# nicolapiccinelli/libmpc

Measured on AMD Instinct MI355X. Metric: MPC solves/sec (whole node) + p50 solve latency, quadrotor LMPC N=20 batch=4096, higher is better.
Workload: dtype f64; 1 GPU; quadrotor_ex.cpp LMPC nx=12 nu=4 ny=12 ph=ch=20, batch 4096 per GPU, SplitMix64 x0/u0/yref (SURVEY 8d), maximum_iteration=250; parallelism=single GPU, rccl_ranks=0, streams=1

## Files before the change

### include/mpcx.h

```cpp
#ifndef MPCX_H
#define MPCX_H

#include <stdint.h>

#ifdef __cplusplus
extern "C" {
#endif

#define MPCX_OK              0
#define MPCX_E_INVALID      -1
#define MPCX_E_UNSUPPORTED  -2
#define MPCX_E_DEVICE       -3
#define MPCX_E_NUMERIC      -4
#define MPCX_E_STATE        -5

#define MPCX_STATUS_SUCCESS        0
#define MPCX_STATUS_MAX_ITERATION  1
#define MPCX_STATUS_INFEASIBLE     2
#define MPCX_STATUS_ERROR          3
#define MPCX_STATUS_UNKNOWN        4

#define MPCX_SOLVER_SOLVED               1
#define MPCX_SOLVER_SOLVED_INACCURATE    2
#define MPCX_SOLVER_MAX_ITER_REACHED    -2
// ... 348 lines not shown
int mpcx_comm_get_unique_id(void *id_out );
int mpcx_comm_create(int device, int rank, int world, const void *id, mpcx_comm_t *out);
int mpcx_comm_destroy(mpcx_comm_t c);
int mpcx_comm_rank(mpcx_comm_t c);
int mpcx_comm_world(mpcx_comm_t c);
int mpcx_allgather_u(mpcx_comm_t c, const double *u_local, int rows_per_rank, int nu, double *u_all, void *stream);

typedef struct mpcx_lmpc_hetero *mpcx_lmpc_hetero_t;
int mpcx_lmpc_hetero_create(const mpcx_lmpc_t *controllers, int count, int device, mpcx_lmpc_hetero_t *out);
int mpcx_lmpc_hetero_create_ex(const mpcx_lmpc_t *controllers, int count, int device, int condense_on_host, mpcx_lmpc_hetero_t *out);
int mpcx_lmpc_hetero_destroy(mpcx_lmpc_hetero_t f);
int mpcx_lmpc_hetero_get_info(mpcx_lmpc_hetero_t f, int *count, int *active_words, int *m_ref, double *bytes_per_model);
int mpcx_lmpc_hetero_solve_batch(mpcx_lmpc_hetero_t f, const mpcx_lmpc_batch *b, const int32_t *model_index, void *stream);
int mpcx_lmpc_hetero_time_solve_batch(mpcx_lmpc_hetero_t f, const mpcx_lmpc_batch *b, const int32_t *model_index, void *stream,
                                      int repeats, float *ms_mean);
int mpcx_lmpc_hetero_sensitivity_batch(mpcx_lmpc_hetero_t f, const mpcx_lmpc_sens *s, const int32_t *model_index, void *stream);
int mpcx_lmpc_hetero_loop_create(mpcx_lmpc_hetero_t f, const mpcx_lmpc_loop_desc *d, const int32_t *model_index, void *stream, mpcx_lmpc_loop_t *out);
int mpcx_lmpc_hetero_loop_create_observed(mpcx_lmpc_hetero_t f, const mpcx_lmpc_loop_desc *d, const mpcx_lmpc_observer_desc *o, const int32_t *model_index,
                                          void *stream, mpcx_lmpc_loop_t *out);
int mpcx_lmpc_hetero_loop_create_offset_free(mpcx_lmpc_hetero_t f, const mpcx_lmpc_loop_desc *d, const mpcx_lmpc_disturbance_observer_desc *o,
                                             const int32_t *model_index, void *stream, mpcx_lmpc_loop_t *out);
int mpcx_lmpc_hetero_loop_create_offset_free_target(mpcx_lmpc_hetero_t f, const mpcx_lmpc_loop_desc *d, const mpcx_lmpc_disturbance_observer_desc *o,
                                                    const mpcx_lmpc_target_desc *t, const int32_t *model_index, void *stream, mpcx_lmpc_loop_t *out);

int mpcx_lmpc_set_total_batch(mpcx_lmpc_t h, int total);

int mpcx_lmpc_debug_time_kernels(mpcx_lmpc_t h, const mpcx_lmpc_batch *b, void *stream, int repeats, float *ms3);
int mpcx_lmpc_debug_get(mpcx_lmpc_t h, const char *name, double *out, int cap);
int mpcx_lmpc_debug_setup_counts(mpcx_lmpc_t h, int *full, int *refs);
int mpcx_lmpc_debug_use_fused(mpcx_lmpc_t h, int mode);
int mpcx_lmpc_debug_force_generic(mpcx_lmpc_t h, int on);
int mpcx_lmpc_debug_set_rounds(mpcx_lmpc_t h, int rounds0, int check_every);
int mpcx_lmpc_debug_set_cycle_buffer(mpcx_lmpc_t h, void *dev_ptr);
int mpcx_lmpc_loop_debug_replay(mpcx_lmpc_loop_t l, void *stream);
int mpcx_lmpc_loop_debug_tick(mpcx_lmpc_loop_t l, int *tick);
int mpcx_nlmpc_loop_debug_replay(mpcx_nlmpc_loop_t l, void *stream);
int mpcx_nlmpc_loop_debug_tick(mpcx_nlmpc_loop_t l, int *tick);
int mpcx_nlmpc_debug_set_tolerances(mpcx_nlmpc_t h, double tol_step, double tol_con);
int mpcx_nlmpc_debug_last_form(void);
int mpcx_dare_debug_product(int product);
int mpcx_nlmpc_last_form(mpcx_nlmpc_t h);
int mpcx_nlmpc_debug_get_ws(mpcx_nlmpc_t h, int instance, double *out, int cap, int *layout, int nlayout);
int mpcx_nlmpc_debug_generated_source(const mpcx_nlmpc_source *src, char *out, int cap);
int mpcx_nlmpc_debug_compile_source(const mpcx_nlmpc_source *src);
int mpcx_lmpc_hetero_debug_get(mpcx_lmpc_hetero_t f, int k, const char *name, double *out, int cap);

const char *mpcx_version(void);

#ifdef __cplusplus
}
#endif
#endif
```

### libmpc_amd/_capi.py

```python
from __future__ import annotations

import ctypes as C
import os

_HERE = os.path.dirname(os.path.abspath(__file__))
LIB_PATH = os.environ.get("MPCX_LIBRARY", os.path.join(_HERE, "libmpcx.so"))

OK = 0
E_INVALID, E_UNSUPPORTED, E_DEVICE, E_NUMERIC, E_STATE = -1, -2, -3, -4, -5
STATUS_SUCCESS, STATUS_MAX_ITERATION, STATUS_INFEASIBLE, STATUS_ERROR, STATUS_UNKNOWN = range(5)
REF_SHARED, REF_PER_INSTANCE, REF_PER_STEP = 0, 1, 2
DARE_CONTROL, DARE_ESTIMATOR = 0, 1
REF_PREVIEW = 3


class Dims(C.Structure):
    _fields_ = [(n, C.c_int) for n in ("nx", "nu", "ndu", "ny", "ph", "ch")]


class LParams(C.Structure):
    _fields_ = [("maximum_iteration", C.c_int), ("time_limit", C.c_double), ("enable_warm_start", C.c_int),
                ("alpha", C.c_double), ("rho", C.c_double), ("eps_rel", C.c_double), ("eps_abs", C.c_double),
                ("eps_prim_inf", C.c_double), ("eps_dual_inf", C.c_double),
                ("verbose", C.c_int), ("adaptive_rho", C.c_int), ("polish", C.c_int)]
# ... 78 lines not shown
    "mpcx_lmpc_set_objective_weights", "mpcx_lmpc_set_objective_weights_slice",
    "mpcx_lmpc_set_state_bounds", "mpcx_lmpc_set_state_bounds_slice",
    "mpcx_lmpc_set_input_bounds", "mpcx_lmpc_set_input_bounds_slice",
    "mpcx_lmpc_set_output_bounds", "mpcx_lmpc_set_output_bounds_slice",
    "mpcx_lmpc_set_input_rate_bounds", "mpcx_lmpc_set_input_rate_bounds_slice",
    "mpcx_lmpc_set_soft_constraint_weights", "mpcx_lmpc_set_soft_constraint_weights_slice",
    "mpcx_lmpc_set_terminal_cost",
    "mpcx_lmpc_set_linear_constraints", "mpcx_lmpc_set_linear_constraints_slice",
    "mpcx_lmpc_set_linear_constraint_weights", "mpcx_lmpc_set_linear_constraint_weights_slice",
    "mpcx_lmpc_set_scalar_constraint_slice", "mpcx_lmpc_set_scalar_constraint_index",
    "mpcx_lmpc_set_references", "mpcx_lmpc_set_references_slice",
    "mpcx_lmpc_set_exogenous_inputs", "mpcx_lmpc_set_exogenous_inputs_slice",
    "mpcx_lmpc_set_optimizer_parameters", "mpcx_lmpc_set_strict_infeasibility", "mpcx_lmpc_setup", "mpcx_lmpc_solve_batch",
    "mpcx_lmpc_time_solve_batch", "mpcx_lmpc_sensitivity_batch", "mpcx_lmpc_sens_size", "mpcx_lmpc_sensitivity_host",
    "mpcx_lmpc_param_sensitivity_batch", "mpcx_lmpc_param_sens_size", "mpcx_lmpc_param_sens_reserve", "mpcx_lmpc_param_sensitivity_host",
    "mpcx_lmpc_model_sensitivity_batch", "mpcx_lmpc_model_sens_size", "mpcx_lmpc_model_sens_reserve", "mpcx_lmpc_model_sensitivity_host", "mpcx_lmpc_solve_host", "mpcx_lmpc_get_info", "mpcx_version",
    "mpcx_lmpc_graph_create", "mpcx_lmpc_graph_launch", "mpcx_lmpc_graph_destroy",
    "mpcx_lmpc_loop_create", "mpcx_lmpc_loop_run", "mpcx_lmpc_loop_destroy", "mpcx_lmpc_loop_desc_size",
    "mpcx_lmpc_loop_create_observed", "mpcx_lmpc_hetero_loop_create_observed", "mpcx_lmpc_observer_desc_size", "mpcx_lmpc_kalman_gain",
    "mpcx_lmpc_loop_create_offset_free", "mpcx_lmpc_hetero_loop_create_offset_free", "mpcx_lmpc_disturbance_observer_desc_size",
    "mpcx_lmpc_loop_create_offset_free_target", "mpcx_lmpc_hetero_loop_create_offset_free_target", "mpcx_lmpc_target_desc_size",
    "mpcx_target_map_batch", "mpcx_target_apply_batch",
    "mpcx_nlmpc_create", "mpcx_nlmpc_destroy", "mpcx_nlmpc_get_dims", "mpcx_nlmpc_evaluate_batch",
    "mpcx_nlparams_default", "mpcx_nlmpc_set_optimizer_parameters", "mpcx_nlmpc_solve_batch", "mpcx_nlmpc_time_solve_batch", "mpcx_discretize_batch", "mpcx_dare_batch",
    "mpcx_nlmpc_set_state_bounds_slice", "mpcx_nlmpc_set_input_bounds_slice", "mpcx_nlmpc_solve_host",
    "mpcx_nlmpc_create_custom", "mpcx_nlmpc_create_from_source", "mpcx_nlmpc_set_input_scale", "mpcx_nlmpc_set_state_scale",
    "mpcx_nlmpc_loop_create", "mpcx_nlmpc_loop_run", "mpcx_nlmpc_loop_destroy", "mpcx_nlmpc_loop_desc_size", "mpcx_nlmpc_plant_step_batch",
    "mpcx_nlmpc_loop_create_observed", "mpcx_nlmpc_ekf_desc_size", "mpcx_nlmpc_ekf_step_batch",
    "mpcx_comm_get_unique_id", "mpcx_comm_create", "mpcx_comm_destroy", "mpcx_comm_rank", "mpcx_comm_world", "mpcx_allgather_u",
    "mpcx_lmpc_hetero_create", "mpcx_lmpc_hetero_destroy", "mpcx_lmpc_hetero_get_info", "mpcx_lmpc_hetero_solve_batch",
    "mpcx_lmpc_hetero_time_solve_batch", "mpcx_lmpc_hetero_create_ex", "mpcx_lmpc_hetero_debug_get", "mpcx_lmpc_hetero_loop_create",
    "mpcx_lmpc_hetero_sensitivity_batch",
    "mpcx_lmpc_set_total_batch", "mpcx_lmpc_debug_time_kernels", "mpcx_lmpc_debug_get", "mpcx_lmpc_debug_setup_counts", "mpcx_lmpc_debug_use_fused",
    "mpcx_lmpc_debug_force_generic", "mpcx_lmpc_debug_set_rounds", "mpcx_lmpc_debug_set_cycle_buffer",
    "mpcx_lmpc_loop_debug_replay", "mpcx_lmpc_loop_debug_tick", "mpcx_nlmpc_loop_debug_replay", "mpcx_nlmpc_loop_debug_tick",
    "mpcx_dare_debug_product", "mpcx_nlmpc_debug_set_tolerances", "mpcx_nlmpc_debug_last_form", "mpcx_nlmpc_last_form", "mpcx_nlmpc_debug_get_ws", "mpcx_nlmpc_debug_generated_source", "mpcx_nlmpc_debug_compile_source",
]


class NLParams(C.Structure):
    _fields_ = [("maximum_iteration", C.c_int), ("time_limit", C.c_double), ("enable_warm_start", C.c_int),
                ("relative_ftol", C.c_double), ("relative_xtol", C.c_double), ("absolute_ftol", C.c_double),
                ("absolute_xtol", C.c_double), ("hard_constraints", C.c_int)]


class NlmpcBatch(C.Structure):
    _fields_ = [("batch", C.c_int), ("x0", C.c_void_p), ("u0", C.c_void_p), ("z_warm", C.c_void_p), ("cmd", C.c_void_p),
                ("cost", C.c_void_p), ("status", C.c_void_p), ("solver_status", C.c_void_p), ("is_feasible", C.c_void_p),
                ("iterations", C.c_void_p), ("z", C.c_void_p), ("seq_state", C.c_void_p), ("seq_input", C.c_void_p),
                ("seq_output", C.c_void_p), ("warm_curvature", C.c_int), ("multipliers", C.c_void_p), ("params", C.c_void_p)]


class NlmpcLoopDesc(C.Structure):
    _fields_ = [("batch", C.c_int), ("ticks", C.c_int), ("x0", C.c_void_p), ("u0", C.c_void_p),
                ("params", C.c_void_p), ("plant_params", C.c_void_p), ("noise", C.c_void_p),
                ("substeps", C.c_int), ("warm", C.c_int),
                ("traj_x", C.c_void_p), ("traj_u", C.c_void_p), ("traj_cost", C.c_void_p),
                ("traj_status", C.c_void_p), ("traj_solver_status", C.c_void_p), ("traj_is_feasible", C.c_void_p),
                ("traj_iterations", C.c_void_p)]


class NlmpcEkfDesc(C.Structure):
    _fields_ = [("ny", C.c_int), ("Cm", C.c_void_p), ("Q", C.c_void_p), ("R", C.c_void_p), ("P0", C.c_void_p),
                ("xhat0", C.c_void_p), ("meas_noise", C.c_void_p), ("traj_xhat", C.c_void_p), ("traj_y", C.c_void_p),
                ("traj_P", C.c_void_p), ("ekf_flags", C.c_void_p)]


# ... 44 lines not shown
        _lib.mpcx_lmpc_hetero_sensitivity_batch.argtypes = [C.c_void_p] * 4
        _lib.mpcx_lmpc_param_sensitivity_batch.argtypes = [C.c_void_p] * 3
        _lib.mpcx_lmpc_param_sens_reserve.argtypes = [C.c_void_p, C.c_int]
        _lib.mpcx_lmpc_param_sensitivity_host.argtypes = [C.c_void_p] * 3 + [C.c_int] + [C.c_void_p] * 7
        _lib.mpcx_lmpc_model_sensitivity_batch.argtypes = [C.c_void_p] * 3
        _lib.mpcx_lmpc_model_sens_reserve.argtypes = [C.c_void_p, C.c_int]
        _lib.mpcx_lmpc_model_sensitivity_host.argtypes = [C.c_void_p] * 3 + [C.c_int] + [C.c_void_p] * 7
        _lib.mpcx_lmpc_graph_create.argtypes = [C.c_void_p, C.c_void_p, C.c_void_p, C.c_void_p]
        _lib.mpcx_lmpc_graph_launch.argtypes = [C.c_void_p, C.c_void_p]
        _lib.mpcx_lmpc_graph_destroy.argtypes = [C.c_void_p]
        _lib.mpcx_lmpc_loop_create.argtypes = [C.c_void_p, C.c_void_p, C.c_void_p, C.c_void_p]
        _lib.mpcx_lmpc_hetero_loop_create.argtypes = [C.c_void_p, C.c_void_p, C.c_void_p, C.c_void_p, C.c_void_p]
        _lib.mpcx_lmpc_loop_create_observed.argtypes = [C.c_void_p] * 5
        _lib.mpcx_lmpc_hetero_loop_create_observed.argtypes = [C.c_void_p] * 6
        _lib.mpcx_lmpc_loop_create_offset_free.argtypes = [C.c_void_p] * 5
        _lib.mpcx_lmpc_hetero_loop_create_offset_free.argtypes = [C.c_void_p] * 6
        _lib.mpcx_lmpc_loop_create_offset_free_target.argtypes = [C.c_void_p] * 6
        _lib.mpcx_lmpc_hetero_loop_create_offset_free_target.argtypes = [C.c_void_p] * 7
        _lib.mpcx_target_map_batch.argtypes = [C.c_int] * 6 + [C.c_void_p] * 9
        _lib.mpcx_target_apply_batch.argtypes = [C.c_int] * 5 + [C.c_void_p, C.c_int] + [C.c_void_p] * 5
        _lib.mpcx_lmpc_kalman_gain.argtypes = [C.c_void_p] * 6
        _lib.mpcx_lmpc_loop_run.argtypes = [C.c_void_p, C.c_void_p]
        _lib.mpcx_lmpc_loop_destroy.argtypes = [C.c_void_p]
        _lib.mpcx_lmpc_loop_debug_replay.argtypes = [C.c_void_p, C.c_void_p]
        _lib.mpcx_lmpc_loop_debug_tick.argtypes = [C.c_void_p, C.c_void_p]
        _lib.mpcx_nlmpc_get_dims.argtypes = [C.c_void_p, C.c_void_p]
        _lib.mpcx_nlmpc_evaluate_batch.argtypes = [C.c_void_p, C.c_int] + [C.c_void_p] * 9
        _lib.mpcx_nlparams_default.restype = None
        for _n in ("mpcx_nlmpc_set_state_bounds_slice", "mpcx_nlmpc_set_input_bounds_slice"):
            getattr(_lib, _n).argtypes = [C.c_void_p, C.c_void_p, C.c_void_p, C.c_int, C.c_int]
        _lib.mpcx_discretize_batch.argtypes = [C.c_int] * 4 + [C.c_void_p] * 3 + [C.c_int] + [C.c_void_p] * 3
        _lib.mpcx_dare_batch.argtypes = [C.c_int] * 5 + [C.c_void_p] * 4 + [C.c_int] * 2 + [C.c_void_p] * 5
        _lib.mpcx_dare_debug_product.argtypes = [C.c_int]
        _lib.mpcx_nlmpc_set_optimizer_parameters.argtypes = [C.c_void_p, C.c_void_p]
        _lib.mpcx_nlmpc_solve_batch.argtypes = [C.c_void_p, C.c_void_p, C.c_void_p]
        _lib.mpcx_nlmpc_time_solve_batch.argtypes = [C.c_void_p, C.c_void_p, C.c_void_p, C.c_int, C.c_void_p]
        _lib.mpcx_nlmpc_create_from_source.argtypes = [C.c_void_p, C.c_double, C.c_int, C.c_void_p]
        _lib.mpcx_nlmpc_set_input_scale.argtypes = [C.c_void_p, C.c_void_p]
        _lib.mpcx_nlmpc_set_state_scale.argtypes = [C.c_void_p, C.c_void_p]
        _lib.mpcx_nlmpc_loop_create.argtypes = [C.c_void_p, C.c_void_p, C.c_void_p, C.c_void_p]
        _lib.mpcx_nlmpc_loop_run.argtypes = [C.c_void_p, C.c_void_p]
        _lib.mpcx_nlmpc_loop_destroy.argtypes = [C.c_void_p]
        _lib.mpcx_nlmpc_loop_debug_replay.argtypes = [C.c_void_p, C.c_void_p]
        _lib.mpcx_nlmpc_loop_debug_tick.argtypes = [C.c_void_p, C.c_void_p]
        _lib.mpcx_nlmpc_plant_step_batch.argtypes = [C.c_void_p, C.c_int] + [C.c_void_p] * 4 + [C.c_int, C.c_void_p, C.c_void_p]
        _lib.mpcx_nlmpc_loop_create_observed.argtypes = [C.c_void_p] * 5
        _lib.mpcx_nlmpc_ekf_step_batch.argtypes = [C.c_void_p, C.c_int] + [C.c_void_p] * 8 + [C.c_int, C.c_int] + [C.c_void_p] * 4
        _lib.mpcx_comm_get_unique_id.argtypes = [C.c_void_p]
        _lib.mpcx_comm_create.argtypes = [C.c_int, C.c_int, C.c_int, C.c_void_p, C.c_void_p]
        _lib.mpcx_comm_destroy.argtypes = [C.c_void_p]
        _lib.mpcx_comm_rank.argtypes = [C.c_void_p]
        _lib.mpcx_comm_world.argtypes = [C.c_void_p]
        _lib.mpcx_allgather_u.argtypes = [C.c_void_p, C.c_void_p, C.c_int, C.c_int, C.c_void_p, C.c_void_p]
    return _lib


def check(rc):
    if rc < 0:
        raise MpcxError(rc, lib().mpcx_last_error().decode())
    return rc
```

### libmpc_amd/csrc/lmpc_device.hpp

```cpp
#pragma once

#include <atomic>
#include <cstdint>
#include <initializer_list>

namespace mpcx {

constexpr int kMaxActive = 28;
constexpr int kSld = kMaxActive + 1;
__host__ __device__ inline int ws_limit(int nz, int mg, int n_soft) { return nz + (n_soft < mg ? n_soft : mg); }
__host__ __device__ inline int ws_capacity(int limit) { return limit > kMaxActive ? limit : kMaxActive; }

struct LmpcDev {
    int nx, nu, ndu, ny, ph, ch, nf, nz, mg;
    int ldz, ldg, ldy;
    int m_ref, neq_ref, active_words;
    int has_dist, n_fixed;
    int max_iter, polish, check_every, polish_rounds0, polish_rounds;
    int cost_direct;
    int cond_status;
    int strict_infeasible;
    int n_soft;
    double alpha, sigma, eps_abs, eps_rel, eps_prim_inf;
    int adaptive_rho; double rho_user;
// ... 49 lines not shown
    const int32_t *model_index;
    long long *dbg_cycles;
};
static_assert(sizeof(LmpcDev) == 712 && sizeof(LmpcBatchDev) == 296, "LmpcDev / LmpcBatchDev changed size: see kernarg_touch (lmpc_fast.hip)");
__host__ __device__ inline size_t lmpc_slot_len(const LmpcDev &m) { const size_t n = (size_t)ws_limit(m.nz, m.mg, m.n_soft); return n * n; }
__host__ __device__ inline int lmpc_model_of(const LmpcBatchDev &Bt, int b) { return Bt.n_models <= 0 ? 0 : (Bt.model_index ? Bt.model_index[b] : b); }

constexpr int kFqCount = 0, kFqTicket = 1, kFqServed = 2, kFqList = 4;
inline size_t lmpc_fallback_queue_bytes(size_t cap) { return (kFqList + cap) * sizeof(int); }
int lmpc_fallback_waves();
int lmpc_fallback_reset(int *fq, void *stream);

size_t lmpc_lds_limit();
int lmpc_kernel_variant(int ldz, int ldg);
struct LmpcScratch { double *ws; size_t cap; int *fq; double *pbuf; int pslots; int *pcounter; };
int lmpc_scratch_reserve(LmpcScratch &s, const LmpcDev &m, int batch, bool with_pcounter, void *stream);
void lmpc_scratch_release(LmpcScratch &s);

enum class LmpcAssemble { Generic, MfmaSharedYref, MfmaInstanceYref };
enum class LmpcForm { TwoKernels, FusedMatvec, Group };
struct LmpcPlan {
    LmpcAssemble assemble;
    LmpcForm form;
    int fused;
};
int lmpc_launch(const LmpcDev &m, const LmpcDev *m_dev, const LmpcBatchDev &b, const LmpcScratch &scratch, void *stream, int which, const LmpcPlan &plan);
int lmpc_fallback_slots(const LmpcDev &m, int batch);
int lmpc_lds_per_wave(const LmpcDev &m, int *stage_len, int *arena_len);
void lmpc_pack_mfma_tiles(const double *src, int rows, int K, double *out);
inline size_t lmpc_packed_len(int rows, int K) { return (size_t)(rows / 16) * ((K + 15) / 16) * 256; }
int lmpc_fast_slice(const LmpcDev &m);
size_t lmpc_group_lds_bytes(const LmpcDev &m);
int lmpc_launch_fast(const LmpcDev &m, const LmpcDev *m_dev, const LmpcBatchDev &b, double *ws, void *stream, LmpcForm form);
struct LmpcLdsCache { std::atomic<size_t> bytes[64]; };
int lmpc_raise_dynamic_lds(LmpcLdsCache &cache, std::initializer_list<const void *> kernels, size_t bytes);
size_t lmpc_condense_lds(const LmpcDev &m, int *NP_out, int *NQ_out, size_t *big_out = nullptr);
int lmpc_condense_launch(LmpcDev *models_d, const LmpcDev &m0, int count, void *stream);

struct LmpcSensArgs {
    int batch;
    bool jacobian;
    const uint32_t *active_lower, *active_upper;
    const int32_t *status;
    const double *seed_cmd, *seed_input;
    double *d_x0, *d_u0, *d_yref;
    int32_t *flags;
};
size_t lmpc_sens_operand(int nz, int kin, int rowsF, const double *MF1, double *out);
int lmpc_sens_launch(const LmpcDev &m, const LmpcDev *m_dev, const double *T0p, const LmpcSensArgs &a, void *stream);

struct LmpcBankSensArgs {
    LmpcSensArgs s;
    const LmpcDev *models;
    const int32_t *model_index;
    int n_models;
};
int lmpc_bank_sens_launch(const LmpcDev &m, const LmpcBankSensArgs &a, void *stream);

struct LmpcParamSensArgs {
    int batch;
    bool reduce;
    const uint32_t *active_lower, *active_upper;
    const int32_t *status;
    const double *seed_cmd, *seed_input;
    const double *u0, *seq_output, *seq_input;
    const double *yref; long yref_bs, yref_ks;
// ... 126 lines not shown
```

### libmpc_amd/csrc/lmpc_fast.hip

```cpp
#include "lmpc_kernel_common.hpp"
#include <cstddef>
#include <cstdlib>
#include <utility>

namespace mpcx {

namespace {

#ifndef MPCX_FAST_PF_MAXCAP
#define MPCX_FAST_PF_MAXCAP 12
#endif
#ifndef MPCX_FAST_RB
#define MPCX_FAST_RB 4
#endif
#ifndef MPCX_FAST_PF
#define MPCX_FAST_PF 4
#endif
#ifndef MPCX_FAST_PF_ALL
#define MPCX_FAST_PF_ALL 6
#endif
#ifndef MPCX_FAST_NBUF
#define MPCX_FAST_NBUF 3
#endif
#ifndef MPCX_FAST_RB_DEEP
// ... 13 lines not shown
#endif
#ifndef MPCX_FAST_XBAR_CHUNK
#define MPCX_FAST_XBAR_CHUNK 0x333442400ull
#endif
constexpr int fast_xbar_chunk(int cap) { return (int)((MPCX_FAST_XBAR_CHUNK >> (4 * (cap / 2))) & 15) > 0 ? (int)((MPCX_FAST_XBAR_CHUNK >> (4 * (cap / 2))) & 15) : 1; }
constexpr bool fast_class_bit(unsigned mask, int cap, int chunks) { return chunks <= MPCX_FAST_XBAR_CHUNKS && ((mask >> (cap / 2)) & 1u) != 0; }
#ifndef MPCX_FAST_STAGE
#define MPCX_FAST_STAGE() __builtin_amdgcn_sched_barrier(0)
#endif
constexpr int kFastCap = 16;
#ifndef MPCX_FAST_ADD_THETA_LATE
#define MPCX_FAST_ADD_THETA_LATE 0.02
#endif
#ifndef MPCX_FAST_SAFE_AFTER
#define MPCX_FAST_SAFE_AFTER 12
#endif

template <int CTRL>
__device__ __forceinline__ double dpp_mov_d(double v)
{
    const int lo = __builtin_amdgcn_mov_dpp(__double2loint(v), CTRL, 0xF, 0xF, true);
    const int hi = __builtin_amdgcn_mov_dpp(__double2hiint(v), CTRL, 0xF, 0xF, true);
    return __hiloint2double(hi, lo);
}
__device__ __forceinline__ double wave_max_dpp(double v)
{
    v = fmax(v, dpp_mov_d<0xB1>(v));
    v = fmax(v, dpp_mov_d<0x4E>(v));
    v = fmax(v, dpp_mov_d<0x141>(v));
    v = fmax(v, dpp_mov_d<0x140>(v));
    v = fmax(v, dpp_mov_d<0x142>(v));
    v = fmax(v, dpp_mov_d<0x143>(v));
    return readlane_d(v, 63);
}

#ifdef MPCX_PROFILE_ROUNDS
#define MPCX_LAP(k) do { const long long now_ = (long long)__builtin_readcyclecounter(); pacc[k] += now_ - plast; plast = now_; } while (0)
#define MPCX_LAP_WAIT(k) do { __builtin_amdgcn_s_waitcnt(0); MPCX_LAP(k); } while (0)
#define MPCX_PROF_ARGS , long long (&pacc)[6], long long &plast
#define MPCX_PROF_PASS , pacc, plast
#else
#define MPCX_LAP(k) do {} while (0)
#define MPCX_LAP_WAIT(k) do {} while (0)
#define MPCX_PROF_ARGS
#define MPCX_PROF_PASS
#endif

template <int CAP, int NLO, int CPZ, int CPG, bool XB = false, bool XL = false>
__device__ __forceinline__ int ws_solve_reg(const gdp gY, const int ldy, const int ldz, const int na, const int lane_in,
                                            const int *wsidx, const double *wsb, const double *t0s, double *lam,
                                            const unsigned (&offz)[CPZ], const unsigned (&offg)[CPG],
                                            double (&wv)[2 * CPZ], double (&gw)[2 * CPG], double &lmax MPCX_PROF_ARGS)
{
    constexpr bool DEEP = CPZ + CPG <= MPCX_FAST_DEEP_CHUNKS;
    constexpr int PF = CAP > MPCX_FAST_PF_MAXCAP ? 0 : (CAP <= (DEEP ? MPCX_FAST_PF_ALL : MPCX_FAST_PF) ? CAP : MPCX_FAST_PF);
    int lane = lane_in;
    asm volatile("" : "+v"(lane));
    const bool real = lane < na;
    const int li = real ? lane : 0;
    const int qi = wsidx[li];
    int qc[CAP];
#pragma unroll
    for (int c = 0; c < CAP; ++c) qc[c] = __builtin_amdgcn_readfirstlane(wsidx[(c < NLO || c < na) ? c : 0]);
    double Sr[CAP];
    const unsigned rowoff = (unsigned)(qi * ldy) * 8u;
    const char MPCX_GAS *const gYb = reinterpret_cast<const char MPCX_GAS *>(gY);
// ... 306 lines not shown

    double w[NZS], f[NZS];
    const double qnan = __builtin_nan("");
#pragma unroll
    for (int c = 0; c < CPZ; ++c) {
        const double2 vf = *reinterpret_cast<const double2 *>(fs + 128 * c + 2 * lane);
        f[2 * c] = vf.x; f[2 * c + 1] = vf.y;
    }
#pragma unroll
    for (int s = 0; s < NZS; ++s) w[s] = infeasible ? qnan : ((128 * (s >> 1) + 2 * lane + (s & 1) < nz) ? wv[s] : 0.0);
    double *stage = fs;
    double cost;
    bool cost_pending = false;
    wave_sync();
#pragma unroll
    for (int c = 0; c < CPZ; ++c) *reinterpret_cast<double2 *>(stage + 128 * c + 2 * lane) = make_double2(w[2 * c], w[2 * c + 1]);
    wave_sync();
    auto soft_penalty = [&]() {
        double pen = 0.0;
#pragma unroll
        for (int s = 0; s < NGS; ++s) {
            const int r = 128 * (s >> 1) + 2 * lane + (s & 1);
            if (r < mg && actg[s] != 0) { const double l = lam[posg[s]]; pen = fma(0.5 * gl(MPCX_G_SOFT(M))[r] * l, l, pen); }
        }
        return pen;
    };
    if (infeasible) {
        cost = 1e30;
    } else if (!M.cost_direct) {
        double j = 0;
#pragma unroll
        for (int s = 0; s < NZS; ++s) j = fma(f[s], w[s], j);
        if (lane < na_last) j = fma(-lam[lane], wsb[lane], j);
        cost = 0.5 * wave_sum(j) + c0;
    } else if (!FUSED && Bt.n_models <= 0) {
#pragma unroll
        for (int c = 0; c < CPZ; ++c) {
            const int e = 128 * c + 2 * lane;
            if (e < ldz) st2(ws + ldz + e, w[2 * c], w[2 * c + 1]);
        }
        if (M.n_soft > 0) {
            const double pen = wave_sum(soft_penalty());
            if (lane == 0) ws[ldz + ldy + 2 * ldg] = c0 + pen;
        }
        cost = 0.0;
        cost_pending = true;
    } else {
        double hw[NZS];
#pragma unroll
        for (int s = 0; s < NZS; ++s) hw[s] = 0;
        matvec_acc<CPZ>(GP(H), ldz, ldz, nz, stage, hw, lane);
        double j = 0;
#pragma unroll
        for (int s = 0; s < NZS; ++s) j += w[s] * (0.5 * hw[s] + f[s]);
        if constexpr (SRC != 1) { if (M.n_soft > 0) j += soft_penalty(); }
        cost = wave_sum(j) + c0;
    }
#pragma unroll
    for (int s = 0; s < NZS; ++s) {
        const int e = 128 * (s >> 1) + 2 * lane + (s & 1);
        if (e < nu) { if (outs) outs[8 + e] = w[s]; else glw(Bt.cmd)[(size_t)b * nu + e] = w[s]; }
    }
    if (outs) {
        if (lane == 0) {
            outs[0] = cost; outs[1] = solver_status == 1 ? 0 : (solver_status == -2 ? 1 : 2); outs[2] = solver_status;
            outs[3] = solver_status == -3 ? 0 : 1; outs[4] = 0; outs[5] = rounds_total; outs[6] = infeasible ? 0 : na_last; outs[7] = 2.0;
        }
    } else if (lane == 0) {
        if (Bt.cost && !cost_pending) glw(Bt.cost)[b] = cost;
        if (Bt.solver_status) glw(Bt.solver_status)[b] = solver_status;
        if (Bt.status) glw(Bt.status)[b] = solver_status == 1 ? 0 : (solver_status == -2 ? 1 : 2);
        if (Bt.is_feasible) glw(Bt.is_feasible)[b] = solver_status == -3 ? 0 : 1;
        if (Bt.iterations) glw(Bt.iterations)[b] = 0;
        if (Bt.polish_rounds) glw(Bt.polish_rounds)[b] = rounds_total;
        if (Bt.active_count) glw(Bt.active_count)[b] = infeasible ? 0 : na_last;
    }

    if (Bt.active_lower && Bt.active_upper) {
        wave_sync();
        unsigned *bl = reinterpret_cast<unsigned *>(t0s);
        unsigned *bu = bl + M.active_words;
        for (int wd = lane; wd < 2 * M.active_words; wd += 64) bl[wd] = 0u;
        wave_sync();
        if (!infeasible) {
#pragma unroll
            for (int s = 0; s < NZS; ++s) {
                const int e = 128 * (s >> 1) + 2 * lane + (s & 1);
                if (e >= nz || actb[s] == 0) continue;
                const double l = lam[posb[s]];
                if (!(fabs(l) > dtol_last)) continue;
                const int side = l < 0 ? -1 : 1;
                const double lo = lws[e], hi = uws[e];
                for (int p = GP(boxrow_ptr)[e]; p < GP(boxrow_ptr)[e + 1]; ++p) {
                    const int rr = GP(boxrow_ref)[p];
                    if (side < 0 && GP(boxrow_lo)[p] == lo) atomicOr(&bl[rr >> 5], 1u << (rr & 31));
                    if (side > 0 && GP(boxrow_hi)[p] == hi) atomicOr(&bu[rr >> 5], 1u << (rr & 31));
                }
            }
#pragma unroll
// ... 633 lines not shown
#pragma unroll
                for (int r = 0; r < 4; ++r) {
                    Bf[(4 * t + r) * 64 + lane] = acc[r];
                    const int row = 16 * t + 4 * r + kq;
                    if (jlive && row < ldz) fj[row] = acc[r];
                }
            } else if (t < ts) {
#pragma unroll
                for (int r = 0; r < 4; ++r) {
                    const int row = 16 * (t - tg) + 4 * r + kq;
                    if (jlive && row < ldg) {
                        const double l0 = PRE ? eblo[r] : GP(lg0)[row], u0 = PRE ? ebhi[r] : GP(ug0)[row];
                        lgj[row] = l0 - acc[r]; ugj[row] = u0 - acc[r];
                    }
                }
            } else if (t < tq) {
#pragma unroll
                for (int r = 0; r < 4; ++r) {
                    const int row = 16 * (t - ts) + 4 * r + kq;
                    if (row < M.ns) badl |= violates(acc[r], PRE ? eblo[r] : GP(slo)[row], PRE ? ebhi[r] : GP(shi)[row], M.eps_abs, M.eps_rel);
                }
            } else {
#pragma unroll
                for (int r = 0; r < 4; ++r) {
                    const int kb2 = 4 * (t - tq) + r;
                    if (kb2 < kin4) c0p = fma(0.5 * Bv[kb2 * 64 + lane], acc[r], c0p);
                }
            }
        };
        int *eqb = reinterpret_cast<int *>(outs + kGroupWaves * outld);
        if (wave < ntile1) tile1.template operator()<true>(wave);
        for (int t = wave + kGroupWaves; t < ntile1; t += kGroupWaves) tile1.template operator()<false>(t);
        if (badl && jlive) atomicOr(&bad[j], 1u);
        c0p += __shfl_xor(c0p, 16, 64);
        c0p += __shfl_xor(c0p, 32, 64);
        if (kq == 0) c0s[wave * 16 + j] = c0p;
        __syncthreads();
        gstamp(5);
#if defined(MPCX_GROUP_CUT) && MPCX_GROUP_CUT == 2
        { return; }
#endif

        auto tile2 = [&]<bool PRE>(const int t) {
            v4d acc = {0.0, 0.0, 0.0, 0.0};
            for (int g0 = 0; g0 < G2; g0 += kGroupG2) {
                v4d a[kGroupG2];
#pragma unroll
                for (int g = 0; g < kGroupG2; ++g) a[g] = (PRE && g0 == 0) ? a2[g] : ld4(Ymp + (((size_t)t * G2 + (g0 + g < G2 ? g0 + g : g0)) * 64 + lane) * 4);
#pragma unroll
                for (int g = 0; g < kGroupG2; ++g)
#pragma unroll
                    for (int e = 0; e < 4; ++e) {
                        const int kb = 4 * (g0 + g) + e;
                        if (kb < nz4) acc = __builtin_amdgcn_mfma_f64_16x16x4f64(a[g][e], Bf[kb * 64 + lane], acc, 0, 0, 0);
                    }
            }
#pragma unroll
            for (int r = 0; r < 4; ++r) {
                const int row = 16 * t + 4 * r + kq;
                if (!jlive) continue;
                if (row < ldz) t0j[row] = acc[r];
                else if (row < ldy) gt0j[row - ldz] = acc[r];
            }
        };
        if (wave < ntile2) tile2.template operator()<true>(wave);
        for (int t = wave + kGroupWaves; t < ntile2; t += kGroupWaves) tile2.template operator()<false>(t);
        if (wave == kGroupWaves - 1) {
            int bits = 0;
// ... 1 lines not shown
            for (int c = 0; c < CPG; ++c) {
                const bool ok = 128 * c + 2 * lane < ldg;
                bits |= ((ok && eql[c].x == equ[c].x) ? 1 : 0) << (2 * c) | ((ok && eql[c].y == equ[c].y) ? 1 : 0) << (2 * c + 1);
            }
            eqb[lane] = bits;
        }
        if (threadIdx.x < kGroupWaves) {
            double *tl = slices + (size_t)threadIdx.x * M.fast_slice + 2 * ZP + 3 * GPD;
            double c0 = 0.0;
            for (int w = 0; w < kGroupWaves; ++w) c0 += c0s[w * 16 + threadIdx.x];
            tl[0] = c0;
            tl[1] = bad[threadIdx.x] ? 1.0 : 0.0;
        }
        __syncthreads();
        const int eqbits = eqb[lane];
        int inst = wave;
#if MPCX_GROUP_BALANCE
        if (b0 + kGroupWaves <= Bt.batch) {
            const double *t0m = mine, *gt0m = mine + ZP, *lgm = gt0m + GPD, *ugm = lgm + GPD;
            auto over = [](double v, double lo, double hi) { return fmax(fmax(lo - v, v - hi), 0.0); };
            double sv = 0.0;
#pragma unroll
            for (int c = 0; c < CPZ; ++c) {
                const int e = 128 * c + 2 * lane;
                const double2 l = *reinterpret_cast<const double2 *>(lwuw + e), u = *reinterpret_cast<const double2 *>(lwuw + ZP + e), t = *reinterpret_cast<const double2 *>(t0m + e);
                sv += over(t.x, l.x, u.x) + over(t.y, l.y, u.y);
            }
#pragma unroll
            for (int c = 0; c < CPG; ++c) {
                const int r = 128 * c + 2 * lane;
                const double2 l = *reinterpret_cast<const double2 *>(lgm + r), u = *reinterpret_cast<const double2 *>(ugm + r), t = *reinterpret_cast<const double2 *>(gt0m + r);
                sv += over(t.x, l.x, u.x) + over(t.y, l.y, u.y);
            }
            sv = wave_sum(sv);
            double *keys = reinterpret_cast<double *>(bad);
            if (lane == 0) keys[wave] = sv;
            __syncthreads();
            const int me = lane & (kGroupWaves - 1), part = lane >> 4;
            const double ki = keys[me];
            int rank = 0;
#pragma unroll
            for (int q = 0; q < kGroupWaves / 4; ++q) {
                const int jj = (kGroupWaves / 4) * part + q;
                const double kj = keys[jj];
                rank += (kj > ki || (kj == ki && jj < me)) ? 1 : 0;
            }
            rank += __shfl_xor(rank, 16, 64);
            rank += __shfl_xor(rank, 32, 64);
            const int q = rank >> 2, sd = (q & 1) ? 3 - (rank & 3) : (rank & 3);
            inst = (int)__builtin_ctzll(__ballot(lane < kGroupWaves && 4 * q + sd == wave));
        }
#endif
        double *const slice_i = slices + (size_t)inst * M.fast_slice;
        const int b = b0 + inst;
        gstamp(6);
#if defined(MPCX_GROUP_CUT) && MPCX_GROUP_CUT == 3
        { return; }
#endif
        if (b < Bt.batch) solve_fast<CPZ, CPG, 2>(M, Bt, b, lane, slice_i, lwuw, glw(wsbase) + (size_t)b * M.wsld, nullptr, outs + inst * outld, eqbits);
        __syncthreads();
        {
            const int t = threadIdx.x;
            if (t < kGroupWaves && b0 + t < Bt.batch) {
                const double *o = outs + t * outld;
                const int bb = b0 + t;
                if (o[7] == 2.0) {
                    if (Bt.cost) glw(Bt.cost)[bb] = o[0];
                    if (Bt.status) glw(Bt.status)[bb] = (int)o[1];
                    if (Bt.solver_status) glw(Bt.solver_status)[bb] = (int)o[2];
                    if (Bt.is_feasible) glw(Bt.is_feasible)[bb] = (int)o[3];
                    if (Bt.iterations) glw(Bt.iterations)[bb] = 0;
                    if (Bt.polish_rounds) glw(Bt.polish_rounds)[bb] = (int)o[5];
                    if (Bt.active_count) glw(Bt.active_count)[bb] = (int)o[6];
                }
            }
            for (int e = t; e < kGroupWaves * nu; e += blockDim.x) {
                const int ti = e / nu, jj = e - ti * nu;
                if (b0 + ti < Bt.batch && outs[ti * outld + 7] == 2.0) glw(Bt.cmd)[(size_t)(b0 + ti) * nu + jj] = outs[ti * outld + 8 + jj];
            }
            if (Bt.fq && t < 64) {
                const bool open = t < kGroupWaves && b0 + t < Bt.batch && outs[t * outld + 7] != 2.0;
                const unsigned long long om = __ballot(open);
                if (om) {
                    int base = 0;
                    if (t == 0) base = atomicAdd(Bt.fq + kFqCount, (int)__builtin_popcountll(om));
                    base = __builtin_amdgcn_readfirstlane(base);
                    const int at = base + (int)__builtin_popcountll(om & ((1ull << t) - 1ull));
                    if (open && at >= 0 && at < Bt.fq_cap) glw(Bt.fq)[kFqList + at] = b0 + t;
                }
            }
        }
    }
}
// ... 37 lines not shown
        static LmpcLdsCache pconf;
        if (lmpc_raise_dynamic_lds(pconf, {reinterpret_cast<const void *>(k5)}, lds_max) != 0) return -3;
        (void)hipMemsetAsync(b.pcounter, 0, 8 * sizeof(int), stream);
        int wgs = (b.batch + kPersistWaves - 1) / kPersistWaves;
        if (wgs > 256) wgs = 256;
        hipLaunchKernelGGL(k5, dim3(wgs), dim3(kPersistWaves * 64), ldsp, stream, m_dev, b, ws, b.pcounter);
    } else if (fused) hipLaunchKernelGGL(k4, dim3(blocks), dim3(kWavesPerBlock * 64), ldsf, stream, m_dev, b, ws);
    else if (b.n_models > 0) hipLaunchKernelGGL(k2h, dim3(blocks), dim3(kWavesPerBlock * 64), ldsf, stream, m_dev, b, ws);
    else hipLaunchKernelGGL(k2, dim3(blocks), dim3(kWavesPerBlock * 64), ldsf, stream, m_dev, b, ws);
    return hipGetLastError() == hipSuccess ? 0 : -3;
}

}

int lmpc_fast_slice(const LmpcDev &m)
{
    const int cp = lmpc_kernel_variant(m.ldz, m.ldg);
    if (cp < 1) return 0;
    const int fixed = cp == 1 ? fast_slice_fixed<1, 1>() : (cp == 2 ? fast_slice_fixed<2, 2>() : fast_slice_fixed<4, 4>());
    const int scratch = m.kin > 2 * m.nx ? m.kin : 2 * m.nx;
    int n = (fixed + scratch + 1) / 2 * 2;
    while (n % 16 != 2) n += 2;
    return n;
}

size_t lmpc_group_lds_bytes(const LmpcDev &m)
{
    const int cp = lmpc_kernel_variant(m.ldz, m.ldg);
    if (cp != 1 && cp != 2) return 0;
    const int nw = cp == 1 ? 16 : 8;
    return ((size_t)2 * 128 * cp + (size_t)nw * m.fast_slice + (size_t)(m.kin / 4 + m.nz16 / 4) * 64 + (size_t)nw * 16 + 16 + (size_t)nw * (8 + ((m.nu + 1) & ~1)) + 32) * sizeof(double);
}

int lmpc_launch_fast(const LmpcDev &m, const LmpcDev *m_dev, const LmpcBatchDev &b, double *ws, void *stream, LmpcForm form)
{
    hipStream_t s = reinterpret_cast<hipStream_t>(stream);
    switch (lmpc_kernel_variant(m.ldz, m.ldg)) {
    case 1: return launch_fast_variant<1, 1>(m, m_dev, b, ws, s, form);
#ifndef MPCX_FAST_ONLY_CP1
    case 2: return launch_fast_variant<2, 2>(m, m_dev, b, ws, s, form);
    case 4: return launch_fast_variant<4, 4>(m, m_dev, b, ws, s, form);
#endif
    default: return -2;
    }
}

}
```

### libmpc_amd/csrc/mpcx_capi.cpp

```cpp
#include <hip/hip_runtime.h>

#include <algorithm>
#include <cmath>
#include <cstdio>
#include <cstring>
#include <memory>
#include <atomic>
#include <chrono>
#include <string>
#include <thread>
#include <type_traits>
#include <vector>

#include "../../include/mpcx.h"
#include "lmpc_device.hpp"
#include "lmpc_model.hpp"

namespace {

thread_local std::string g_err;

int fail(int code, const std::string &msg)
{
    g_err = msg;
// ... 2094 lines not shown
    return MPCX_OK;
}

int mpcx_lmpc_set_total_batch(mpcx_lmpc_t h, int total)
{
    CHECK_H(h);
    if (total < 0) return fail(MPCX_E_INVALID, "negative batch");
    h->total_batch = total;
    return MPCX_OK;
}

int mpcx_lmpc_debug_force_generic(mpcx_lmpc_t h, int on)
{
    CHECK_H(h);
    h->force_generic = on != 0;
    return MPCX_OK;
}

int mpcx_lmpc_debug_set_rounds(mpcx_lmpc_t h, int rounds0, int check_every)
{
    CHECK_H(h);
    h->dbg_rounds0 = rounds0; h->dbg_check_every = check_every;
    h->dirty = true;
    return MPCX_OK;
}

int mpcx_lmpc_debug_set_cycle_buffer(mpcx_lmpc_t h, void *dev_ptr)
{
    CHECK_H(h);
    h->dbg_cycles = static_cast<long long *>(dev_ptr);
    return MPCX_OK;
}

int mpcx_lmpc_debug_get(mpcx_lmpc_t h, const char *name, double *out, int cap)
{
    CHECK_H(h);
    int rc = mpcx_lmpc_setup(h);
    if (rc != MPCX_OK) return rc;
    const auto &o = h->cond;
    const std::vector<double> *v = nullptr;
    std::vector<double> tmp;
    std::string n(name ? name : "");
    if (n == "H") v = &o.H; else if (n == "Kinv") v = &o.Kinv; else if (n == "Gr") v = &o.Gr;
    else if (n == "Gc") v = &o.Gc; else if (n == "Y") v = &o.Y; else if (n == "lw") v = &o.lw;
    else if (n == "uw") v = &o.uw; else if (n == "rho_b") v = &o.rho_b; else if (n == "lg0") v = &o.lg0;
    else if (n == "ug0") v = &o.ug0; else if (n == "rho_g") v = &o.rho_g; else if (n == "g_soft") v = &o.g_soft;
    else if (n == "dims") {
        tmp = {(double)o.nz, (double)o.mg, (double)o.ldz, (double)o.ldg, (double)o.ldy, (double)o.nf,
               (double)o.n_ref, (double)o.m_ref, (double)o.neq_ref, (double)o.fixed_rows.size(),
               (double)h->dev.lds_per_wave, (double)(o.h_regularised ? 1 : 0)};
        v = &tmp;
    } else if (n == "MA0") v = &o.MA[0]; else if (n == "MA1") v = &o.MA[1]; else if (n == "Ym") v = &o.Ym;
    else if (n == "MA0p" || n == "MA1p" || n == "Ymp") {
        const std::vector<double> &src = n == "Ymp" ? o.Ym : o.MA[n == "MA1p" ? 1 : 0];
        const int rows = n == "Ymp" ? o.ldy16 : o.rowsA, K = n == "Ymp" ? o.nz16 : o.kin;
        if (!src.empty()) { tmp.resize(mpcx::lmpc_packed_len(rows, K)); mpcx::lmpc_pack_mfma_tiles(src.data(), rows, K, tmp.data()); }
        v = &tmp;
    } else if (n == "flags") {
        tmp = {(double)h->dev.cost_direct, (double)h->dev.group_ok, (double)h->dev.fused_ok};
        v = &tmp;
    } else if (n == "dims_maps") {
        tmp = {(double)o.kin, (double)o.nxp, (double)o.nup, (double)o.nyp, (double)o.ione, (double)o.nz16, (double)o.mg16,
               (double)o.ns, (double)o.ns16, (double)o.kq16, (double)o.rowsA, (double)o.ldy16};
        v = &tmp;
    } else if (n == "g_refrow") { tmp.assign(o.g_refrow.begin(), o.g_refrow.end()); v = &tmp; }
    else if (n == "MF1") v = &o.MF[1];
// ... 49 lines not shown
```

Measured before the change: 125.6 million solves/s.

## Use permlane/DPP wave reductions and batch final cost evaluation across group via MFMA

Replaces shuffle-based wave sums with gfx950 permlane16/32 swap and DPP sequences for row and full-wave reductions. For the CPZ=2 grouped path, each instance's quadratic cost is no longer reduced inside the per-instance solve. It is deferred and computed after the solves by four waves using MFMA over H times the solution for all group instances, then added into the output. This cuts per-solve reduction latency and serial cost work, but adds an extra synchronisation phase and H reads. A debug probe kernel is added to validate the reduction variants.

```diff
diff --git a/include/mpcx.h b/include/mpcx.h
--- a/include/mpcx.h
+++ b/include/mpcx.h
@@ -404,6 +404,7 @@
 int mpcx_lmpc_debug_force_generic(mpcx_lmpc_t h, int on);
 int mpcx_lmpc_debug_set_rounds(mpcx_lmpc_t h, int rounds0, int check_every);
 int mpcx_lmpc_debug_set_cycle_buffer(mpcx_lmpc_t h, void *dev_ptr);
+int mpcx_lmpc_debug_wave_reduce(const double *in, double *out, int nvec, void *stream);
 int mpcx_lmpc_loop_debug_replay(mpcx_lmpc_loop_t l, void *stream);
 int mpcx_lmpc_loop_debug_tick(mpcx_lmpc_loop_t l, int *tick);
 int mpcx_nlmpc_loop_debug_replay(mpcx_nlmpc_loop_t l, void *stream);
diff --git a/libmpc_amd/_capi.py b/libmpc_amd/_capi.py
--- a/libmpc_amd/_capi.py
+++ b/libmpc_amd/_capi.py
@@ -134,7 +134,7 @@
     "mpcx_lmpc_hetero_time_solve_batch", "mpcx_lmpc_hetero_create_ex", "mpcx_lmpc_hetero_debug_get", "mpcx_lmpc_hetero_loop_create",
     "mpcx_lmpc_hetero_sensitivity_batch",
     "mpcx_lmpc_set_total_batch", "mpcx_lmpc_debug_time_kernels", "mpcx_lmpc_debug_get", "mpcx_lmpc_debug_setup_counts", "mpcx_lmpc_debug_use_fused",
-    "mpcx_lmpc_debug_force_generic", "mpcx_lmpc_debug_set_rounds", "mpcx_lmpc_debug_set_cycle_buffer",
+    "mpcx_lmpc_debug_force_generic", "mpcx_lmpc_debug_set_rounds", "mpcx_lmpc_debug_set_cycle_buffer", "mpcx_lmpc_debug_wave_reduce",
     "mpcx_lmpc_loop_debug_replay", "mpcx_lmpc_loop_debug_tick", "mpcx_nlmpc_loop_debug_replay", "mpcx_nlmpc_loop_debug_tick",
     "mpcx_dare_debug_product", "mpcx_nlmpc_debug_set_tolerances", "mpcx_nlmpc_debug_last_form", "mpcx_nlmpc_last_form", "mpcx_nlmpc_debug_get_ws", "mpcx_nlmpc_debug_generated_source", "mpcx_nlmpc_debug_compile_source",
 ]
@@ -245,6 +245,7 @@
         _lib.mpcx_discretize_batch.argtypes = [C.c_int] * 4 + [C.c_void_p] * 3 + [C.c_int] + [C.c_void_p] * 3
         _lib.mpcx_dare_batch.argtypes = [C.c_int] * 5 + [C.c_void_p] * 4 + [C.c_int] * 2 + [C.c_void_p] * 5
         _lib.mpcx_dare_debug_product.argtypes = [C.c_int]
+        _lib.mpcx_lmpc_debug_wave_reduce.argtypes = [C.c_void_p, C.c_void_p, C.c_int, C.c_void_p]
         _lib.mpcx_nlmpc_set_optimizer_parameters.argtypes = [C.c_void_p, C.c_void_p]
         _lib.mpcx_nlmpc_solve_batch.argtypes = [C.c_void_p, C.c_void_p, C.c_void_p]
         _lib.mpcx_nlmpc_time_solve_batch.argtypes = [C.c_void_p, C.c_void_p, C.c_void_p, C.c_int, C.c_void_p]
diff --git a/libmpc_amd/csrc/lmpc_device.hpp b/libmpc_amd/csrc/lmpc_device.hpp
--- a/libmpc_amd/csrc/lmpc_device.hpp
+++ b/libmpc_amd/csrc/lmpc_device.hpp
@@ -105,6 +105,7 @@
 int lmpc_fast_slice(const LmpcDev &m);
 size_t lmpc_group_lds_bytes(const LmpcDev &m);
 int lmpc_launch_fast(const LmpcDev &m, const LmpcDev *m_dev, const LmpcBatchDev &b, double *ws, void *stream, LmpcForm form);
+int lmpc_debug_wave_reduce(const double *in, double *out, int nvec, void *stream);
 struct LmpcLdsCache { std::atomic<size_t> bytes[64]; };
 int lmpc_raise_dynamic_lds(LmpcLdsCache &cache, std::initializer_list<const void *> kernels, size_t bytes);
 size_t lmpc_condense_lds(const LmpcDev &m, int *NP_out, int *NQ_out, size_t *big_out = nullptr);
diff --git a/libmpc_amd/csrc/lmpc_fast.hip b/libmpc_amd/csrc/lmpc_fast.hip
--- a/libmpc_amd/csrc/lmpc_fast.hip
+++ b/libmpc_amd/csrc/lmpc_fast.hip
@@ -69,6 +69,89 @@
     v = fmax(v, dpp_mov_d<0x142>(v));
     v = fmax(v, dpp_mov_d<0x143>(v));
     return readlane_d(v, 63);
+}
+#ifndef MPCX_FAST_DPP_SUMS
+#define MPCX_FAST_DPP_SUMS 1
+#endif
+template <bool ROW16>
+__device__ __forceinline__ double lane_swap_pair_sum(double v)
+{
+    const unsigned lo = (unsigned)__double2loint(v), hi = (unsigned)__double2hiint(v);
+    if constexpr (ROW16) {
+        const auto l = __builtin_amdgcn_permlane16_swap(lo, lo, false, false);
+        const auto h = __builtin_amdgcn_permlane16_swap(hi, hi, false, false);
+        return __hiloint2double((int)h[0], (int)l[0]) + __hiloint2double((int)h[1], (int)l[1]);
+    } else {
+        const auto l = __builtin_amdgcn_permlane32_swap(lo, lo, false, false);
+        const auto h = __builtin_amdgcn_permlane32_swap(hi, hi, false, false);
+        return __hiloint2double((int)h[0], (int)l[0]) + __hiloint2double((int)h[1], (int)l[1]);
+    }
+}
+template <bool ROW16>
+__device__ __forceinline__ int lane_swap_pair_sum(int v)
+{
+    if constexpr (ROW16) { const auto r = __builtin_amdgcn_permlane16_swap((unsigned)v, (unsigned)v, false, false); return (int)(r[0] + r[1]); }
+    else { const auto r = __builtin_amdgcn_permlane32_swap((unsigned)v, (unsigned)v, false, false); return (int)(r[0] + r[1]); }
+}
+__device__ __forceinline__ double wave_sum_full(double v)
+{
+    v = lane_swap_pair_sum<false>(v);
+    v = lane_swap_pair_sum<true>(v);
+    v += dpp_mov_d<0x128>(v);
+    {
+        int lo = __builtin_amdgcn_mov_dpp(__double2loint(v), 0x12C, 0xF, 0x5, true);
+        int hi = __builtin_amdgcn_mov_dpp(__double2hiint(v), 0x12C, 0xF, 0x5, true);
+        lo = __builtin_amdgcn_update_dpp(lo, __double2loint(v), 0x124, 0xF, 0xA, false);
+        hi = __builtin_amdgcn_update_dpp(hi, __double2hiint(v), 0x124, 0xF, 0xA, false);
+        v += __hiloint2double(hi, lo);
+    }
+    v += dpp_mov_d<0x4E>(v);
+    v += dpp_mov_d<0xB1>(v);
+    return v;
+}
+template <typename T>
+__device__ __forceinline__ T wave_sum_rows_swap(T v)
+{
+    v = lane_swap_pair_sum<true>(v);
+    return lane_swap_pair_sum<false>(v);
+}
+template <typename T>
+__device__ __forceinline__ T wave_sum_rows_shfl(T v)
+{
+    v += __shfl_xor(v, 16, 64);
+    v += __shfl_xor(v, 32, 64);
+    return v;
+}
+template <typename T>
+__device__ __forceinline__ T wave_sum_rows(T v)
+{
+#if MPCX_FAST_DPP_SUMS
+    return wave_sum_rows_swap(v);
+#else
+    return wave_sum_rows_shfl(v);
+#endif
+}
+__device__ __forceinline__ double wave_sum_any(double v)
+{
+#if MPCX_FAST_DPP_SUMS
+    v += dpp_mov_d<0xB1>(v);
+    v += dpp_mov_d<0x4E>(v);
+    v += dpp_mov_d<0x141>(v);
+    v += dpp_mov_d<0x140>(v);
+    v += dpp_mov_d<0x142>(v);
+    v += dpp_mov_d<0x143>(v);
+    return readlane_d(v, 63);
+#else
+    return wave_sum(v);
+#endif
+}
+__device__ __forceinline__ double wave_sum_cost(double v)
+{
+#if MPCX_FAST_DPP_SUMS
+    return wave_sum_full(v);
+#else
+    return wave_sum(v);
+#endif
 }
 
 #ifdef MPCX_PROFILE_ROUNDS
@@ -441,7 +524,7 @@
 #pragma unroll
         for (int s = 0; s < NZS; ++s) j = fma(f[s], w[s], j);
         if (lane < na_last) j = fma(-lam[lane], wsb[lane], j);
-        cost = 0.5 * wave_sum(j) + c0;
+        cost = 0.5 * wave_sum_cost(j) + c0;
     } else if (!FUSED && Bt.n_models <= 0) {
 #pragma unroll
         for (int c = 0; c < CPZ; ++c) {
@@ -449,10 +532,13 @@
             if (e < ldz) st2(ws + ldz + e, w[2 * c], w[2 * c + 1]);
         }
         if (M.n_soft > 0) {
-            const double pen = wave_sum(soft_penalty());
+            const double pen = wave_sum_cost(soft_penalty());
             if (lane == 0) ws[ldz + ldy + 2 * ldg] = c0 + pen;
         }
         cost = 0.0;
+        cost_pending = true;
+    } else if (SRC == 2 && CPZ == 2 && Bt.n_models <= 0) {
+        cost = M.n_soft > 0 ? c0 + wave_sum_cost(soft_penalty()) : c0;
         cost_pending = true;
     } else {
         double hw[NZS];
@@ -463,7 +549,7 @@
 #pragma unroll
         for (int s = 0; s < NZS; ++s) j += w[s] * (0.5 * hw[s] + f[s]);
         if constexpr (SRC != 1) { if (M.n_soft > 0) j += soft_penalty(); }
-        cost = wave_sum(j) + c0;
+        cost = wave_sum_cost(j) + c0;
     }
 #pragma unroll
     for (int s = 0; s < NZS; ++s) {
@@ -473,7 +559,7 @@
     if (outs) {
         if (lane == 0) {
             outs[0] = cost; outs[1] = solver_status == 1 ? 0 : (solver_status == -2 ? 1 : 2); outs[2] = solver_status;
-            outs[3] = solver_status == -3 ? 0 : 1; outs[4] = 0; outs[5] = rounds_total; outs[6] = infeasible ? 0 : na_last; outs[7] = 2.0;
+            outs[3] = solver_status == -3 ? 0 : 1; outs[4] = cost_pending ? 1.0 : 0.0; outs[5] = rounds_total; outs[6] = infeasible ? 0 : na_last; outs[7] = 2.0;
         }
     } else if (lane == 0) {
         if (Bt.cost && !cost_pending) glw(Bt.cost)[b] = cost;
@@ -1173,8 +1259,7 @@
         if (wave < ntile1) tile1.template operator()<true>(wave);
         for (int t = wave + kGroupWaves; t < ntile1; t += kGroupWaves) tile1.template operator()<false>(t);
         if (badl && jlive) atomicOr(&bad[j], 1u);
-        c0p += __shfl_xor(c0p, 16, 64);
-        c0p += __shfl_xor(c0p, 32, 64);
+        c0p = wave_sum_rows(c0p);
         if (kq == 0) c0s[wave * 16 + j] = c0p;
         __syncthreads();
         gstamp(5);
@@ -1242,7 +1327,7 @@
                 const double2 l = *reinterpret_cast<const double2 *>(lgm + r), u = *reinterpret_cast<const double2 *>(ugm + r), t = *reinterpret_cast<const double2 *>(gt0m + r);
                 sv += over(t.x, l.x, u.x) + over(t.y, l.y, u.y);
             }
-            sv = wave_sum(sv);
+            sv = wave_sum_any(sv);
             double *keys = reinterpret_cast<double *>(bad);
             if (lane == 0) keys[wave] = sv;
             __syncthreads();
@@ -1255,8 +1340,7 @@
                 const double kj = keys[jj];
                 rank += (kj > ki || (kj == ki && jj < me)) ? 1 : 0;
             }
-            rank += __shfl_xor(rank, 16, 64);
-            rank += __shfl_xor(rank, 32, 64);
+            rank = wave_sum_rows(rank);
             const int q = rank >> 2, sd = (q & 1) ? 3 - (rank & 3) : (rank & 3);
             inst = (int)__builtin_ctzll(__ballot(lane < kGroupWaves && 4 * q + sd == wave));
         }
@@ -1269,6 +1353,59 @@
 #endif
         if (b < Bt.batch) solve_fast<CPZ, CPG, 2>(M, Bt, b, lane, slice_i, lwuw, glw(wsbase) + (size_t)b * M.wsld, nullptr, outs + inst * outld, eqbits);
         __syncthreads();
+        if constexpr (CPZ == 2) {
+            if (M.cost_direct && Bt.n_models <= 0) {
+                double *cs = c0s;
+                if (wave < 4) {
+                    const int ntile = M.nz16 >> 4;
+                    const gdp H = GP(H), Hp = GP(Hp);
+                    constexpr int kCostGB = 4;
+                    double part = 0.0;
+                    for (int tl = wave; tl < ntile; tl += 4) {
+                        v4d acc = {0.0, 0.0, 0.0, 0.0};
+                        auto wop = [&](const int kb) { const int k = 4 * kb + kq; return k < M.nz ? fj[k] : 0.0; };
+                        if (Hp) {
+                            for (int g0 = 0; g0 < G2; g0 += kCostGB) {
+                                v4d a[kCostGB];
+#pragma unroll
+                                for (int g = 0; g < kCostGB; ++g) if (g0 + g < G2) a[g] = ld4(Hp + (((size_t)tl * G2 + g0 + g) * 64 + lane) * 4);
+#pragma unroll
+                                for (int g = 0; g < kCostGB; ++g)
+#pragma unroll
+                                    for (int e = 0; e < 4; ++e) {
+                                        const int kb = 4 * (g0 + g) + e;
+                                        if (kb < nz4) acc = __builtin_amdgcn_mfma_f64_16x16x4f64(a[g][e], wop(kb), acc, 0, 0, 0);
+                                    }
+                            }
+                        } else {
+                            const int rowa = 16 * tl + j;
+                            const gdp Ht = H + (rowa < ldz ? rowa : 0);
+                            for (int kb = 0; kb < nz4; ++kb) {
+                                const int col = 4 * kb + kq;
+                                const double a = (col < M.nz && rowa < ldz) ? Ht[(size_t)col * ldz] : 0.0;
+                                acc = __builtin_amdgcn_mfma_f64_16x16x4f64(a, wop(kb), acc, 0, 0, 0);
+                            }
+                        }
+#pragma unroll
+                        for (int r = 0; r < 4; ++r) {
+                            const int row = 16 * tl + 4 * r + kq;
+                            const double w = wop(4 * tl + r);
+                            const double fr = row < M.nz ? Bf[(4 * tl + r) * 64 + lane] : 0.0;
+                            part = fma(w, 0.5 * acc[r] + fr, part);
+                        }
+                    }
+                    part = wave_sum_rows(part);
+                    if (kq == 0) cs[wave * 16 + j] = part;
+                }
+                __syncthreads();
+                if (threadIdx.x < kGroupWaves) {
+                    double *o = outs + threadIdx.x * outld;
+                    const int t = threadIdx.x;
+                    if (o[7] == 2.0 && o[4] == 1.0) o[0] = ((cs[t] + cs[16 + t]) + (cs[32 + t] + cs[48 + t])) + o[0];
+                }
+                __syncthreads();
+            }
+        }
         {
             const int t = threadIdx.x;
             if (t < kGroupWaves && b0 + t < Bt.batch) {
@@ -1372,6 +1509,26 @@
     return ((size_t)2 * 128 * cp + (size_t)nw * m.fast_slice + (size_t)(m.kin / 4 + m.nz16 / 4) * 64 + (size_t)nw * 16 + 16 + (size_t)nw * (8 + ((m.nu + 1) & ~1)) + 32) * sizeof(double);
 }
 
+namespace {
+__global__ __launch_bounds__(64) void lmpc_wave_reduce_probe(const double *in, double *out)
+{
+    const int lane = threadIdx.x;
+    const double x = in[(size_t)blockIdx.x * 64 + lane];
+    double *o = out + (size_t)blockIdx.x * 256;
+    o[lane] = wave_sum(x);
+    o[64 + lane] = wave_sum_full(x);
+    o[128 + lane] = wave_sum_rows_shfl(x);
+    o[192 + lane] = wave_sum_rows_swap(x);
+}
+}
+
+int lmpc_debug_wave_reduce(const double *in, double *out, int nvec, void *stream)
+{
+    if (nvec <= 0) return 0;
+    hipLaunchKernelGGL(lmpc_wave_reduce_probe, dim3(nvec), dim3(64), 0, reinterpret_cast<hipStream_t>(stream), in, out);
+    return hipGetLastError() == hipSuccess ? 0 : -3;
+}
+
 int lmpc_launch_fast(const LmpcDev &m, const LmpcDev *m_dev, const LmpcBatchDev &b, double *ws, void *stream, LmpcForm form)
 {
     hipStream_t s = reinterpret_cast<hipStream_t>(stream);
diff --git a/libmpc_amd/csrc/mpcx_capi.cpp b/libmpc_amd/csrc/mpcx_capi.cpp
--- a/libmpc_amd/csrc/mpcx_capi.cpp
+++ b/libmpc_amd/csrc/mpcx_capi.cpp
@@ -2150,6 +2150,12 @@
     return MPCX_OK;
 }
 
+int mpcx_lmpc_debug_wave_reduce(const double *in, double *out, int nvec, void *stream)
+{
+    if (!in || !out || nvec < 0) return fail(MPCX_E_INVALID, "mpcx_lmpc_debug_wave_reduce: null buffer or negative count");
+    return mpcx::lmpc_debug_wave_reduce(in, out, nvec, stream) == 0 ? MPCX_OK : fail(MPCX_E_DEVICE, "mpcx_lmpc_debug_wave_reduce: launch failed");
+}
+
 int mpcx_lmpc_debug_get(mpcx_lmpc_t h, const char *name, double *out, int cap)
 {
     CHECK_H(h);
```

Measured after the change: 128.3 million solves/s (median of 6 runs). 2.1% higher.
